# hucsmn/suffix_array

Measured on AMD Instinct MI355X. Metric: input MB/s indexed (SA build), higher is better.
Workload: dtype u8; 1 GPU; c3_english_256m: 268435456 bytes per GPU, seed base + rank, one independent text per GPU; n_bytes=268435456, sigma=57, symbols_per_key=13, refinement_rounds=9, text_rounds=0, radix_passes=25, unresolved_after_initial_sort=199000237

## Files before the change

### suffix_array_amd/csrc/host/pipeline.hpp

```cpp
#pragma once
#include "support.hpp"
#include "tuning.hpp"
#include "pool.hpp"

#include <functional>

namespace sa {

constexpr int SORT_MAX_WG = 1024;
constexpr int BK_TOP_BITS_MAX = 18;
constexpr uint32_t BK_BUCKETS_MAX = 1u << BK_TOP_BITS_MAX;
static_assert(32 - 16 <= BK_MAX_LBITS, "two 8-bit passes inside a bucket");
constexpr size_t GRAM_MAX_ENTRIES = (size_t)1 << 24;
static_assert(GROUP_CAP_MAX == GS_CAP, "Tuning clamps SA_AMD_GROUP_CAP to the kernel's cap");

#ifdef SA_AMD_DIAG
typedef void (*DownsweepFn)(const uint64_t *, const uint32_t *, uint64_t *, uint32_t *, uint32_t *,
                            const uint32_t *, int64_t, int, uint32_t, int64_t, int);
struct SortVariant { int threads, items, wg_per_cu; DownsweepFn fn; const char *name; };
static const SortVariant sort_variants[] = {
    { 1024, 8, 2, k_radix_downsweep_wcl<1024, 8, 16, 1, false, uint64_t, 4>, "carry-completed lines 1024x8 + LDS prefetch of half of the next tile's keys (default)" },
    { 1024, 8, 2, k_radix_downsweep_wcl<1024, 8>, "carry-completed lines 1024x8" },
    { 512, 16, 1, k_radix_downsweep_wcl<512, 16>, "carry-completed lines 512x16" },
    { 1024, 8, 2, k_radix_downsweep_wcl<1024, 8, 8>, "carry 1024x8, granule 8" },
// ... 24 lines not shown
}

#else
constexpr int N_SORT_VARIANTS = 1;
#endif

struct SortScratch {
    uint32_t *spine;
    uint32_t *digit_tot;
    unsigned long long *status;
    uint32_t *err;
};

struct Workspace {
    uint64_t *keysA, *keysB, *keysC;
    uint32_t *valsA, *valsB, *isa, *U0, *U1, *G0, *G1;
    uint32_t *spine, *digit_tot, *tcnt, *thead, *tnext, *hist, *total, *chg, *has_isa;
    uint8_t *packed;
    uint8_t *gram_flags;
    uint4 *gram_table;
    uint32_t *surv_bits, *surv_cnt, *todo_bits, *ft_cnt, *ft_head;
    unsigned long long *os_status;
    uint32_t *os_err;
    uint32_t *bk_start;
    uint32_t *early_bits, *early_cnt;
    SortScratch ss;
    size_t bytes, bytes2;
};

static Workspace carve(void *base, int64_t n, size_t cap = ~(size_t)0, void *base2 = nullptr)
{
    Workspace w;
    const size_t N = (size_t)(n > 0 ? n : 1);
    size_t off = 0, off2 = 0;
    auto take = [&](size_t b) {
        if (off + b <= cap) { size_t o = off; off = align_up(off + b, 256); return (char *)base + o; }
        size_t o = off2; off2 = align_up(off2 + b, 256); return (char *)base2 + o;
    };
    const size_t rr_tiles = (size_t)ceil_div((int64_t)N, RR_TILE);
    const size_t ft_tiles = (size_t)ceil_div((int64_t)N, FT_TILE) + 1;
    const size_t gram_entries = N < GRAM_MAX_ENTRIES ? N : GRAM_MAX_ENTRIES;
    w.spine = (uint32_t *)take((size_t)RADIX * SORT_MAX_WG * 4);
    w.digit_tot = (uint32_t *)take(RADIX * 4);
    w.os_status = (unsigned long long *)take(((size_t)ceil_div((int64_t)N, OS_MIN_TILE) + 1) * RADIX * 8);
    w.os_err = (uint32_t *)take(256);
    w.hist = (uint32_t *)take(256 * 4);
    w.total = (uint32_t *)take(256);
    w.chg = (uint32_t *)take((size_t)RR_CHG_COUNTERS * 32 * 4);
    w.tcnt = (uint32_t *)take(rr_tiles * 4);
    w.thead = (uint32_t *)take(rr_tiles * 4);
    w.tnext = (uint32_t *)take(rr_tiles * 4);
    w.surv_cnt = (uint32_t *)take(rr_tiles * 4);
    w.ft_cnt = (uint32_t *)take(ft_tiles * 4);
    w.ft_head = (uint32_t *)take(ft_tiles * 4);
    w.bk_start = (uint32_t *)take(((size_t)BK_BUCKETS_MAX + 1) * 4);
    w.early_cnt = (uint32_t *)take(((N + 1 + EARLY_TILE - 1) / EARLY_TILE + 8) * 4);
    w.gram_table = (uint4 *)take((gram_entries / 64 + 1) * 16);
    w.has_isa = (uint32_t *)take((N + 31) / 32 * 4);
    w.surv_bits = (uint32_t *)take((N + 31) / 32 * 4);
    w.todo_bits = (uint32_t *)take((N + 31) / 32 * 4);
    w.early_bits = (uint32_t *)take(((N + 1 + 31) / 32 + EARLY_THREADS) * 4);
    w.gram_flags = (uint8_t *)take(gram_entries + 64);
    w.packed = (uint8_t *)take(N / 2 + 64);
    w.keysA = (uint64_t *)take((N + 64) * 8);
    w.keysB = (uint64_t *)take((N + 64) * 8);
    w.valsA = (uint32_t *)take(N * 4);
    w.valsB = (uint32_t *)take(N * 4);
    w.isa = (uint32_t *)take(N * 4);
// ... 965 lines not shown
    int64_t threshold = 0;
    std::function<void(hipEvent_t)> start;
    std::function<int64_t()> stop;
    bool started = false;
    int64_t m_snap = 0;
    int64_t covered = 0;
    int64_t holes = 0;
    const uint32_t *d_bits = nullptr, *d_tile_off = nullptr, *d_holes = nullptr;
    hipEvent_t ev = nullptr;
};

struct DeviceBuild {
    const uint8_t *dT;
    uint32_t *dSA, *SA;
    int64_t n;
    hipStream_t st;
    Tuning tn;
    Workspace w;
    sa_amd_stats local;
    EarlyDownload *early = nullptr;
    bool trace = false;
    double trace_t = 0;
    double lap() { const double t = now_ms(), d = t - trace_t; trace_t = t; return d; }
    bool timing_only() const
    {
#ifdef SA_AMD_DIAG
        return tn.timing_only_initial_sort;
#else
        return false;
#endif
    }
    KeyParams P, Ptext;
    int sigma = 0, key_bits = 0, g_bits = 0, top_shift = 0;
    bool force_dense = false, text_ok = false, local_ok = false, probe_dense = false;
    SortResult sr;
    const uint32_t *sorted32 = nullptr;
    int bucket_top_bits = 0;
    bool flat_text = false;
    bool bucket_finished = false;
    uint64_t *sorted0 = nullptr;
    uint32_t *Ucur = nullptr, *Unext = nullptr, *Gcur = nullptr, *Gnext = nullptr, *Vcur = nullptr;
    uint64_t *rkA = nullptr, *rkB = nullptr;
    int64_t tiles = 0, m = 0, depth = 0;
    uint32_t m32 = 0;
    bool lists_ready = false, finished32 = false, fused64 = false, sparse = false;
    bool isa_tail_ranks = false;
// ... 482 lines not shown
        m = m32;
        local.unresolved_after_initial = m;
        if (timing_only()) m = 0;
        }
        return SA_AMD_OK;
    }

    int finish_top32_ties()
    {
        int rc = SA_AMD_OK; (void)rc;
        if (!finished32 && top_shift && m > 0) {
            rkA = (sr.keys == w.keysA) ? w.keysB : w.keysA;
            rkB = w.keysC;
            PROF(KC_RR_APPLY, n, st, hipLaunchKernelGGL((k_rr_apply<true, false, 1, uint32_t>), dim3((unsigned)tiles), dim3(RR_THREADS), 0, st,
                                                        sorted32, (const uint32_t *)SA, (const uint32_t *)nullptr, n,
                                                        (const uint32_t *)w.tcnt, (const uint32_t *)w.thead, SA, w.isa, Ucur, Gcur, Vcur, 0u,
                                                        w.has_isa, 0, (uint64_t *)nullptr, (uint32_t *)nullptr, (const uint32_t *)w.total, 0, (const uint32_t *)nullptr, 0, (uint32_t *)nullptr));
            uint32_t *Valt = (Vcur == w.valsA) ? w.valsB : w.valsA;
            Refined rf;
            KeySrc K = KeySrc(); K.mode = KS_LOWKEY; K.kb = top_shift;
            rc = refine_list(rkA, rkB, Vcur, Valt, Ucur, Gcur, Unext, Gnext, m, n, dT, P, K, g_bits, &local_ok, w, st, &local, &rf, tn);
            if (rc) return rc;
            tiles = ceil_div(m, RR_TILE);
            PROF(KC_RR_COUNT, m, st, hipLaunchKernelGGL((k_rr_count<false>), dim3((unsigned)tiles), dim3(RR_THREADS), 0, st, rf.keys,
                                                        (const uint32_t *)Ucur, m, w.tcnt, w.thead, 0, (uint32_t *)nullptr, 0));
            PROF(KC_RR_SCAN, tiles, st, hipLaunchKernelGGL((k_rr_scan), dim3(1), dim3(SPINE_THREADS), 0, st, w.tcnt, w.thead, tiles, w.total));
            PROF(KC_RR_APPLY, m, st, hipLaunchKernelGGL((k_rr_apply<false, true, 3>), dim3((unsigned)tiles), dim3(RR_THREADS), 0, st,
                                                        rf.keys, rf.vals, (const uint32_t *)Ucur, m, (const uint32_t *)w.tcnt,
                                                        (const uint32_t *)w.thead, SA, w.isa, Unext, Gnext, rf.vnext, (uint32_t)n,
                                                        (uint32_t *)nullptr, 0, (uint64_t *)nullptr, (uint32_t *)nullptr,
                                                        (const uint32_t *)w.total, 0, (const uint32_t *)nullptr, 0, (uint32_t *)nullptr));
            { const int rcw = read_words(&m32, w.total, 4, st); if (rcw) return rcw; }
            m = m32;
            uint32_t *t;
            t = Ucur; Ucur = Unext; Unext = t;
            t = Gcur; Gcur = Gnext; Gnext = t;
            Vcur = rf.vnext;
            lists_ready = true;
            local.unresolved_after_initial = m;
        }
        return SA_AMD_OK;
    }

    int rank_setup_and_text_rounds()
    {
        int rc = SA_AMD_OK; (void)rc;
        key2_bits = bit_length((uint64_t)(2 * n));
        const int64_t sparse_div = tn.sparse_div;
        const int64_t sparse_limit = n / sparse_div;
        sparse = false;
        const bool dense_first = m > 0 && !lists_ready && (force_dense || (!text_ok && m > sparse_limit) || (probe_dense && m > sparse_limit));
        if (m > 0 && dense_first) {
            isa_tail_ranks = !tn.no_first_tail;
            if (isa_tail_ranks)
// ... 39 lines not shown
                PROF(KC_RR_APPLY, n, st, hipLaunchKernelGGL((k_rr_apply<true, false, 1>), dim3((unsigned)tiles), dim3(RR_THREADS), 0, st,
                                                            (const uint64_t *)sorted0, (const uint32_t *)SA, (const uint32_t *)nullptr, n,
                                                            (const uint32_t *)w.tcnt, (const uint32_t *)w.thead, SA, w.isa, Ucur, Gcur, Vcur, 0u,
                                                            w.has_isa, 0, (uint64_t *)nullptr, (uint32_t *)nullptr, (const uint32_t *)w.total, 0, (const uint32_t *)nullptr, 0, (uint32_t *)nullptr));
            }
            bool progressing = true;

            bool counters_clear = false;
            while (text_ok && s_sym > 0 && m > sparse_limit && local.text_rounds < tn.max_text_rounds && progressing) {
                if ((rc = early_maybe_start())) return rc;
                const int64_t m_before = m;
                uint32_t *Valt = (Vcur == w.valsA) ? w.valsB : w.valsA;
                Refined rf;
                KeySrc K = KeySrc(); K.mode = KS_TEXT; K.h = depth; K.s = s_sym; K.kb = tkb;
                RoundCtl ctl;
                ctl.defer = prev_clean && local_ok && !tn.no_defer;
                ctl.counters_clear = counters_clear;
                rc = refine_list(rkA, rkB, Vcur, Valt, Ucur, Gcur, Unext, Gnext, m, n, dT, Ptext, K, g_bits, &local_ok, w, st, &local, &rf, tn, false, nullptr, &ctl);
                if (rc) return rc;
                uint32_t words[RC_WORDS];
                for (int attempt = 0; ; ++attempt) {
                    const uint32_t *gate = ctl.deferred ? (const uint32_t *)(w.total + RC_FLAGGED) : (const uint32_t *)nullptr;
                    tiles = ceil_div(m, RR_TILE);
                    PROF(KC_RR_COUNT, m, st, hipLaunchKernelGGL((k_rr_count<false>), dim3((unsigned)tiles), dim3(RR_THREADS), 0, st, rf.keys,
                                                                (const uint32_t *)Ucur, m, w.tcnt, w.thead, 0, (uint32_t *)nullptr, 0, gate));
                    PROF(KC_RR_SCAN, tiles, st, hipLaunchKernelGGL((k_rr_scan_round), dim3(2), dim3(SPINE_THREADS), 0, st, w.tcnt, w.thead, tiles, w.total,
                                                                   (uint32_t *)nullptr, (uint32_t *)nullptr, w.total + RC_BIG_LISTED, gate));
                    PROF(KC_RR_APPLY, m, st, hipLaunchKernelGGL((k_rr_apply<false, true, 3>), dim3((unsigned)tiles), dim3(RR_THREADS), 0, st,
                                                                rf.keys, rf.vals, (const uint32_t *)Ucur, m, (const uint32_t *)w.tcnt,
                                                                (const uint32_t *)w.thead, SA, w.isa, Unext, Gnext, rf.vnext,
                                                                (uint32_t)n, (uint32_t *)nullptr, 0, (uint64_t *)nullptr, (uint32_t *)nullptr,
                                                                (const uint32_t *)w.total, 0, (const uint32_t *)nullptr, 0, (uint32_t *)nullptr, gate));
                    { const int rcw = read_words(words, w.total, sizeof(words), st); if (rcw) return rcw; }
                    if (!ctl.deferred) break;
                    if (words[RC_FLAGGED] == 0) { ctl.m_flagged = 0; local.locally_sorted += m; break; }
                    if (attempt > 0) return SA_AMD_EINTERNAL;
                    uint32_t tot[RC_WORDS];
                    memcpy(tot, words, sizeof(tot));
                    ctl.resume_tot = tot; ctl.defer = false; ctl.deferred = false;
                    rc = refine_list(rkA, rkB, Vcur, Valt, Ucur, Gcur, Unext, Gnext, m, n, dT, Ptext, K, g_bits, &local_ok, w, st, &local, &rf, tn, false, nullptr, &ctl);
                    if (rc) return rc;
                    ctl.resume_tot = nullptr;
                }
                prev_clean = ctl.m_flagged == 0;
                counters_clear = true;
                uint32_t *Vnext = rf.vnext;
                m32 = words[0];
                m = m32;
                uint32_t *t;
                t = Ucur; Ucur = Unext; Unext = t;
                t = Gcur; Gcur = Gnext; Gnext = t;
                Vcur = Vnext;
                depth += s_sym;
                local.text_rounds++;
                local.rounds++;
// ... 47 lines not shown
            KeySrc K = KeySrc();
            K.mode = sparse ? KS_SPARSE : KS_RANK; K.h = h; K.kb = key2_bits; K.isa = w.isa;
            if (!local_ok && !tn.no_local_sort && m * 2 < m_local_off) local_ok = true;
            const bool retry_local = !local_ok && ++rounds_local_off >= 3;
            K.iters = (!sparse && local_ok && chase_ok) ? (m >= tn.chase_big_min ? tn.chase_big : tn.chase) : 1;
            if (K.iters > 1) K.mode = KS_CHASE;
            K.has_isa = w.has_isa; K.sorted_keys = sorted0; K.sorted_top32 = sorted32; K.sa = SA; K.depth = depth_text; K.top_shift = top_shift;
            Refined rf;
            if (local_ok) { m_local_off = m; rounds_local_off = 0; }
            const int64_t expect = (!parent_tail || m < changed_prev) ? m : changed_prev;
            const bool bin = !sparse && binned(n, expect, tn);
            RoundCtl ctl;
            ctl.defer = prev_clean && !bin && local_ok && !tn.no_defer;
            ctl.skip_big = all_small;
            ctl.counters_clear = counters_clear;
            rc = refine_list(rkA, rkB, Vcur, Valt, Ucur, Gcur, Unext, Gnext, m, n, dT, P, K, g_bits, &local_ok, w, st, &local, &rf, tn, retry_local, &split_rest, &ctl);
            if (rc) return rc;
            uint32_t words[64 + RR_CHG_COUNTERS * 32];
            for (int attempt = 0; ; ++attempt) {
                if (retry_local && rf.m_global < m) { m_local_off = m; rounds_local_off = 0; }
                const uint64_t *keysS = rf.keys; const uint32_t *valsS = rf.vals; uint32_t *Vnext = rf.vnext;
                const uint32_t *gate = ctl.deferred ? (const uint32_t *)(w.total + RC_FLAGGED) : (const uint32_t *)nullptr;
                tiles = ceil_div(m, RR_TILE);
                if (sparse)
                    PROF(KC_RR_COUNT, m, st, hipLaunchKernelGGL((k_rr_count<false>), dim3((unsigned)tiles), dim3(RR_THREADS), 0, st, keysS, Ucur, m, w.tcnt,
                                       w.thead, 0, (uint32_t *)nullptr, 0, gate));
                else
                    PROF(KC_RR_COUNT, m, st, hipLaunchKernelGGL((k_rr_count<false, uint64_t, true>), dim3((unsigned)tiles), dim3(RR_THREADS), 0, st, keysS, Ucur, m,
                                       w.tcnt, w.thead, 0, w.tnext, key2_bits, gate));
                PROF(KC_RR_SCAN, tiles, st, hipLaunchKernelGGL((k_rr_scan_round), dim3(2), dim3(SPINE_THREADS), 0, st, w.tcnt, w.thead, tiles, w.total,
                                                               sparse ? (uint32_t *)nullptr : w.tnext, sparse ? (uint32_t *)nullptr : w.chg, w.total + RC_BIG_LISTED, gate));
                if (sparse) {
                    PROF(KC_RR_APPLY, m, st, hipLaunchKernelGGL((k_rr_apply<false, true, 1>), dim3((unsigned)tiles), dim3(RR_THREADS), 0, st,
                                                                keysS, valsS, Ucur, m, w.tcnt, w.thead, SA, w.isa, Unext, Gnext, Vnext,
                                                                (uint32_t)n, w.has_isa, key2_bits, (uint64_t *)nullptr, (uint32_t *)nullptr, (const uint32_t *)w.total, 0, (const uint32_t *)nullptr, 0, (uint32_t *)nullptr, gate));
                } else if (bin) {
                    uint64_t *pk = (keysS == rkA) ? rkB : rkA;
                    PROF(KC_RR_APPLY, m, st, hipLaunchKernelGGL((k_rr_apply<false, true, 2>), dim3((unsigned)tiles), dim3(RR_THREADS), 0, st,
                                                                keysS, valsS, Ucur, m, w.tcnt, w.thead, SA, w.isa, Unext, Gnext, Vnext,
                                                                (uint32_t)n, (uint32_t *)nullptr, key2_bits, pk, Gcur, (const uint32_t *)w.total, 0,
                                                                (const uint32_t *)w.tnext, parent_tail ? 1 : 0, w.chg, (const uint32_t *)nullptr, sa_final));
                    { const int rcw = read_words(words, w.total, sizeof(words), st); if (rcw) return rcw; }
                    int64_t pairs = 0;
                    for (int c = 0; c < RR_CHG_COUNTERS; ++c) pairs += words[64 + c * 32];
                    if (pairs > 0) {
                        rc = scatter_binned((uint32_t *)pk, Gcur, (uint32_t *)keysS, (uint32_t *)valsS, pairs, n, w, st, &local, tn);
                        if (rc) return rc;
                    }
                    break;
                } else {
                    PROF(KC_RR_APPLY, m, st, hipLaunchKernelGGL((k_rr_apply<false, true, 0>), dim3((unsigned)tiles), dim3(RR_THREADS), 0, st,
                                                                keysS, valsS, Ucur, m, w.tcnt, w.thead, SA, w.isa, Unext, Gnext, Vnext,
                                                                (uint32_t)n, (uint32_t *)nullptr, key2_bits, (uint64_t *)nullptr,
                                                                (uint32_t *)nullptr, (const uint32_t *)w.total, 0,
                                                                (const uint32_t *)w.tnext, parent_tail ? 1 : 0, w.chg, gate, sa_final));
                }
                { const int rcw = read_words(words, w.total, sparse ? (size_t)RC_WORDS * 4 : sizeof(words), st); if (rcw) return rcw; }
                if (!ctl.deferred) break;
                if (words[RC_FLAGGED] == 0) {
                    ctl.m_flagged = 0;
                    ctl.big_listed = ctl.skip_big ? -1 : (int64_t)words[RC_BIG_LISTED_SAVED];
                    rf.m_global = words[RC_BIG_ORDERED_SAVED];
                    local.locally_sorted += m;
                    break;
                }
                if (attempt > 0) return SA_AMD_EINTERNAL;
                uint32_t tot[RC_WORDS];
                memcpy(tot, words, sizeof(tot));
                ctl.resume_tot = tot; ctl.defer = false; ctl.deferred = false;
                rc = refine_list(rkA, rkB, Vcur, Valt, Ucur, Gcur, Unext, Gnext, m, n, dT, P, K, g_bits, &local_ok, w, st, &local, &rf, tn, retry_local, &split_rest, &ctl);
                if (rc) return rc;
                ctl.resume_tot = nullptr;
                ++deferred_misses;
            }
            uint32_t *Vnext = rf.vnext;
            prev_clean = ctl.m_flagged == 0;
            if (prev_clean && (ctl.big_listed == 0 || m <= GS_CAP)) all_small = true;
            counters_clear = true;
            {
// ... 39 lines not shown
        PROF(KC_MISC, 1, st, hipLaunchKernelGGL((k_set_u32), dim3(1), dim3(1), 0, st, dSA, 0u));
        HIP_TRY(hipStreamSynchronize(st));
        if (stats) *stats = local;
        return SA_AMD_OK;
    }
    B.w = dWork2 ? carve(dWork, n, (size_t)work_bytes, dWork2) : carve(dWork, n);
    const Workspace &w = B.w;
    if ((int64_t)w.bytes > work_bytes || (int64_t)w.bytes2 > work2_bytes) return SA_AMD_EINVAL;
    if (n <= tn.small_max) {
        if (n <= SM_LITE_SINGLE_N)
            PROF(KC_MISC, n, st, hipLaunchKernelGGL((k_small_sa_lite), dim3(1), dim3(SM_LITE_THREADS), 0, st, dT, dSA, (int)n, w.total));
        else
            PROF(KC_MISC, n, st, hipLaunchKernelGGL((k_small_sa), dim3(1), dim3(SM_THREADS), 0, st, dT, dSA, (int)n, w.total));
        uint32_t rounds = 0;
        { const int rcw = read_words(&rounds, w.total, 4, st); if (rcw) return rcw; }
        local.rounds = (int)rounds;
        local.readbacks = g_readbacks;
        g_prof.resolve();
        g_last_stats = local;
        if (stats) *stats = local;
        return SA_AMD_OK;
    }
    HIP_TRY(hipMemsetAsync(w.os_err, 0, 16, st));
    int rc;
    if ((rc = B.geometry_and_probes())) return rc;
    if (!B.unary_done) {
    if ((rc = B.initial_sort())) return rc;
    if ((rc = B.first_round_from_sorted_keys())) return rc;
    if ((rc = B.group_heads())) return rc;
    if ((rc = B.finish_top32_ties())) return rc;
    if ((rc = B.rank_setup_and_text_rounds())) return rc;
    if ((rc = B.doubling_rounds())) return rc;
    }
    if ((rc = B.early_finish())) return rc;
    hipLaunchKernelGGL(k_set_u32, dim3(1), dim3(1), 0, st, dSA, (uint32_t)n);
    LAUNCH_CHECK(st);
    {
        uint32_t gave_up[4] = { 0, 0, 0, 0 };
        const int rcw = read_words(gave_up, w.os_err, 16, st); if (rcw) return rcw;
        if (gave_up[0] || gave_up[3]) return SA_AMD_EINTERNAL;
    }
    local.readbacks = g_readbacks;
    if (B.trace) fprintf(stderr, "suffix_array_amd: %d blocking read-backs in this build (%d rounds deferred their mid-round count and had to run the global sort after all)\n", g_readbacks, B.deferred_misses);
    g_prof.resolve();
    g_last_stats = local;
    if (stats) *stats = local;
// ... 5 lines not shown
```

### suffix_array_amd/csrc/host/tuning.hpp

```cpp
#pragma once
#include <cstdlib>
#include <cstdint>
#include <atomic>

namespace sa {

constexpr int64_t SPARSE_DIV_DEFAULT = 64;
constexpr int GROUP_CAP_MAX = 1024;

constexpr int UNBWT_SPACING_DEFAULT = 256;
constexpr int UNBWT_SPACING_MAX = 65536;
constexpr int UNBWT_SPACING_MIN = 4;
constexpr int UNBWT_CAP_DEFAULT = 4096;
constexpr int UNBWT_CAP_MAX = 1 << 24;
constexpr int UNBWT_RESTART_WALKS = 64;

inline bool env_flag(const char *name)
{
    const char *e = getenv(name);
    return e && *e && !(e[0] == '0' && e[1] == 0);
}

inline int64_t env_int(const char *name, int64_t def, int64_t lo, int64_t hi)
{
// ... 14 lines not shown
struct Tuning {
    int sort_variant = 0;
    int sort32_variant = 0;
    int key_bits_max = 64;
    int group_cap = GROUP_CAP_MAX;
    int64_t sparse_div = SPARSE_DIV_DEFAULT;
    bool sparse_div_set = false;
    bool force_dense = false;
    bool no_text_rounds = false;
    bool no_local_sort = false;
    bool no_top32 = false;
    bool force_top32 = false;
    bool no_fused_finish = false;
    bool fused64 = false;
    bool no_packed_text = false;
    bool no_binned_isa = false;
    bool binned_isa_always = false;
    bool no_run_skip = false;
    int64_t run_skip_min = (int64_t)1 << 25;
    int64_t dense_rekey_min = (int64_t)1 << 22;
    bool no_first_tail = false;
    bool sa_every_round = false;
    bool setup_key_copy = false;
    bool no_repeat_probe = false;
    int64_t binned_min = (int64_t)1 << 26;
    int chase = 7;
    int chase_big = 3;
    int64_t chase_big_min = (int64_t)1 << 23;
    int scatter_levels = 0;
    int max_text_rounds = 4;
    bool no_split = false;
    int64_t split_min = (int64_t)1 << 22;
    int64_t split_group_min = (int64_t)1 << 15;
    bool no_gram_keys = false;
    int64_t gram_min_n = (int64_t)1 << 22;
    int gram_g = 0;
    int gram_tail_max = 8;
    int top32_partners_x100 = 50;
    int top32_collisions_x100 = 400;
    int64_t top32_probe_min_n = (int64_t)1 << 21;
    int small_max = 8192;
    bool no_onesweep = false;
    int onesweep_flags = 0;
    int onesweep64_shape = 0;
    int onesweep32_shape = 0;
    bool no_unary_shortcut = false;
// ... 80 lines not shown
        t.count_next_below_n = env_int("SA_AMD_COUNT_NEXT_BELOW_N", 393216, 0, (int64_t)1 << 40);
        t.no_unary_shortcut = env_flag("SA_AMD_NO_UNARY_SHORTCUT");

        t.no_text_keys = env_flag("SA_AMD_NO_TEXT_KEYS");
        t.no_value_bits = env_flag("SA_AMD_NO_VALUE_BITS");
        t.no_bucket_sort = env_flag("SA_AMD_NO_BUCKET_SORT");
        t.bucket_min_n = env_int("SA_AMD_BUCKET_MIN_N", (int64_t)1 << 25, 1, (int64_t)1 << 40);
        t.no_bucket_finish = env_flag("SA_AMD_NO_BUCKET_FINISH");
        t.bucket_finish_always = env_flag("SA_AMD_BUCKET_FINISH_ALWAYS");
        t.bucket_bits = (int)env_int("SA_AMD_BUCKET_BITS", 0, 0, 18);
        if (t.bucket_bits != 16 && t.bucket_bits != 18) t.bucket_bits = 0;
        t.bucket_shape = (int)env_int("SA_AMD_BUCKET_SHAPE", -1, -1, 64);
#ifdef SA_AMD_DIAG
        t.sample_sort = env_flag("SA_AMD_SAMPLE_SORT");
        t.sample_merge = env_flag("SA_AMD_SAMPLE_MERGE");
        t.sample_sort_min_n = env_int("SA_AMD_SAMPLE_SORT_MIN_N", (int64_t)1 << 26, (int64_t)1 << 17, (int64_t)1 << 40);
        t.sample_log = (int)env_int("SA_AMD_SAMPLE_LOG", 0, 0, 24);
        if (t.sample_log != 0 && t.sample_log < 16) t.sample_log = 16;
        t.timing_only_initial_sort = env_flag("SA_AMD_TIMING_ONLY_INITIAL_SORT");
        {
            const int r = g_rerank_routes.load(std::memory_order_relaxed);
            t.sa_every_round = (r & 1) != 0;
            t.setup_key_copy = (r & 2) != 0;
        }
#endif
        return t;
    }
};

constexpr size_t STAGE_BYTES = (size_t)16 << 20;

struct HostTuning {
    int small_max;
    int copy_threads;
    size_t staged_min;
    bool prefault;
    int prefault_keep;
    bool prefault_wait;
    int64_t early_div;
    size_t early_min;
    size_t early_chunk;
    int64_t early_wait;
    bool reduced;
    bool lanes;
    int64_t lanes_min_n;
    bool kernel_d2h;
// ... 28 lines not shown
```

### suffix_array_amd/csrc/kernels/onesweep.hpp

```cpp
#pragma once
#include "common.hpp"
#include "radix_sort.hpp"

namespace sa {

constexpr int OS_NSEG = 8;
constexpr int OS_LB = 3;
struct __attribute__((packed, aligned(4))) Words4 { uint32_t x, y, z, w; };
constexpr int OS_MIN_TILE = 4096;

__device__ __forceinline__ unsigned os_xcc_id()
{
    return (unsigned)__builtin_amdgcn_s_getreg((3 << 11) | 20) & 7u;
}

typedef __attribute__((address_space(1))) unsigned long long os_gu64;

__device__ __forceinline__ uint32_t text_key32(const uint8_t *__restrict__ T, int64_t n, int64_t i)
{
    if (i + 8 <= n) {
        const uintptr_t a = (uintptr_t)(T + i);
        const uint32_t *W = (const uint32_t *)(a & ~(uintptr_t)3);
        const uint32_t lo = W[0], hi = W[1];
        const uint32_t le = __builtin_amdgcn_alignbyte(hi, lo, (uint32_t)(a & 3u));
        return __builtin_bswap32(le);
    }
    uint32_t k = 0;
#pragma unroll
    for (int b = 0; b < 4; ++b) k = (k << 8) | (i + b < n ? (uint32_t)T[i + b] : 0u);
    return k;
}

__global__ __launch_bounds__(SORT_THREADS) void k_text_upsweep32(const uint8_t *__restrict__ T, int64_t n, uint32_t *__restrict__ counts,
                                                                 int shift, uint32_t dmask, int64_t chunk_elems, int G, int split, int64_t sub_elems)
{
    __shared__ uint32_t h[SORT_WAVES][512];
    for (int i = threadIdx.x; i < SORT_WAVES * 512; i += SORT_THREADS) (&h[0][0])[i] = 0;
    __syncthreads();
    uint32_t *mine = h[wave_id()];
// ... 456 lines not shown
```

### suffix_array_amd/csrc/kernels/rerank.hpp

```cpp
#pragma once
#include "common.hpp"

namespace sa {

constexpr int RR_THREADS = 1024;
constexpr int RR_ITEMS = 8;
constexpr int RR_TILE = RR_THREADS * RR_ITEMS;

constexpr int RR_WAVE_ELEMS = WAVE * RR_ITEMS;

struct WaveGroups { uint64_t head[RR_ITEMS], tied[RR_ITEMS], valid[RR_ITEMS], phead[RR_ITEMS]; };

__device__ __forceinline__ uint64_t shfl64(uint64_t v, int src)
{
    return ((uint64_t)(uint32_t)__shfl((int)(uint32_t)(v >> 32), src, WAVE) << 32) | (uint32_t)__shfl((int)(uint32_t)v, src, WAVE);
}

template <typename KeyT, bool PARENTS = false>
__device__ __forceinline__ WaveGroups rr_wave_classify(const KeyT *__restrict__ keys, int64_t m, int64_t wbase, int key_shift, int g_shift = 0,
                                                       uint64_t *kout = nullptr)
{
    const int l = lane_id();
    uint64_t k[RR_ITEMS];
    WaveGroups g;
// ... 180 lines not shown
{
    rr_scan_body(tile_cnt, tile_head, tiles, out_total);
}

__global__ __launch_bounds__(SPINE_THREADS) void k_rr_scan_pair(uint32_t *__restrict__ cntA, uint32_t *__restrict__ headA, uint32_t *__restrict__ outA,
                                                                 uint32_t *__restrict__ cntB, uint32_t *__restrict__ headB, uint32_t *__restrict__ outB,
                                                                 int64_t tiles)
{
    if (blockIdx.x == 0) rr_scan_body(cntA, headA, tiles, outA);
    else rr_scan_body(cntB, headB, tiles, outB);
}

__global__ __launch_bounds__(SPINE_THREADS) void k_rr_scan_round(uint32_t *__restrict__ tile_cnt, uint32_t *__restrict__ tile_head, int64_t tiles,
                                                                  uint32_t *__restrict__ out_total, uint32_t *__restrict__ tile_first,
                                                                  uint32_t *__restrict__ changed_cnt, uint32_t *__restrict__ clear2,
                                                                  const uint32_t *__restrict__ gate)
{
    if (gate && *gate) return;
    if (blockIdx.x == 0) { rr_scan_body(tile_cnt, tile_head, tiles, out_total); return; }
    if (tile_first) rr_scan_next_body(tile_first, tiles, changed_cnt);
    if (threadIdx.x == 0 && clear2) { clear2[2] = clear2[0]; clear2[3] = clear2[1]; clear2[0] = 0u; clear2[1] = 0u; }
}

template <bool FIRST, bool WRITE_SA, int ISA_MODE, typename KeyT = uint64_t, bool FTAIL = false>
__global__ __launch_bounds__(RR_THREADS) void k_rr_apply(
    const KeyT *__restrict__ keys, const uint32_t *__restrict__ V, const uint32_t *__restrict__ U, int64_t m,
    const uint32_t *__restrict__ tile_cnt, const uint32_t *__restrict__ tile_head, uint32_t *__restrict__ SA,
    uint32_t *__restrict__ ISA, uint32_t *__restrict__ Uo, uint32_t *__restrict__ Go, uint32_t *__restrict__ Vo,
    uint32_t n_text, uint32_t *__restrict__ has_isa, int g_shift, uint64_t *__restrict__ pair_k,
    uint32_t *__restrict__ pair_v, const uint32_t *__restrict__ tile_total, int key_shift,
    const uint32_t *__restrict__ tile_next, int parent_tail, uint32_t *__restrict__ changed_cnt,
    const uint32_t *__restrict__ gate = nullptr,
    int sa_final = 0)
{
    constexpr bool SPARSE = ISA_MODE == 1;
    if (gate && *gate) return;
    constexpr bool TAIL = (FIRST ? FTAIL : true) && (ISA_MODE == 0 || ISA_MODE == 2);
    constexpr bool COUNT_CHANGED = TAIL && !FIRST;
    constexpr int NW = RR_THREADS / WAVE;
    __shared__ uint32_t wcnt[NW], whead[NW], wfirst[NW];
    __shared__ uint32_t s_chg;
    if (COUNT_CHANGED && threadIdx.x == 0) s_chg = 0;
    if (FIRST && !WRITE_SA && SPARSE) {
        const uint32_t here = tile_cnt[blockIdx.x];
        const uint32_t next = (blockIdx.x + 1 < gridDim.x) ? tile_cnt[blockIdx.x + 1] : *tile_total;
        if (next == here) return;
    }
    const int l = lane_id(), w = wave_id();
    const int64_t wbase = (int64_t)blockIdx.x * RR_TILE + (int64_t)w * RR_WAVE_ELEMS;
    const WaveGroups g = rr_wave_classify<KeyT, TAIL>(keys, m, wbase, key_shift, g_shift);
    uint32_t slot[RR_ITEMS], v[RR_ITEMS];
#pragma unroll
    for (int r = 0; r < RR_ITEMS; ++r) {
        const int64_t i = wbase + 64 * r + l;
        const bool in = i < m;
        slot[r] = FIRST ? (uint32_t)i : (in ? U[i] : 0u);
        v[r] = in ? V[i] : 0u;
    }
    {
        uint32_t cnt = 0, lasthead = 0;
#pragma unroll
        for (int r = 0; r < RR_ITEMS; ++r) {
            cnt += (uint32_t)__popcll(g.tied[r]);
            if (g.head[r]) lasthead = (uint32_t)__shfl((int)slot[r], 63 - __builtin_clzll(g.head[r]), WAVE) + 1u;
        }
        if (l == 0) { wcnt[w] = cnt; whead[w] = lasthead; wfirst[w] = TAIL ? rr_first_head_code(g, wbase, 0) : RR_NO_HEAD; }
    }
    __syncthreads();
    uint32_t run_cnt = tile_cnt[blockIdx.x], run_head = tile_head[blockIdx.x];
    for (int ww = 0; ww < w; ++ww) { run_cnt += wcnt[ww]; run_head = run_head > whead[ww] ? run_head : whead[ww]; }
    uint32_t next_code[RR_ITEMS];
    uint32_t n_changed = 0;
    if (TAIL) {
        uint32_t behind = tile_next[blockIdx.x];
        for (int ww = NW - 1; ww > w; --ww) behind = wfirst[ww] != RR_NO_HEAD ? wfirst[ww] : behind;
        if (behind == RR_NO_HEAD) behind = ((uint32_t)m << 1) | 1u;
#pragma unroll
        for (int r = RR_ITEMS - 1; r >= 0; --r) {
            next_code[r] = behind;
            if (g.head[r]) {
                const int b = __builtin_ctzll(g.head[r]);
                behind = ((uint32_t)(wbase + 64 * r + b) << 1) | (uint32_t)((g.phead[r] >> b) & 1ull);
            }
        }
    }
    const uint64_t le_mask = (l == 63) ? ~0ull : ((2ull << l) - 1ull);
    const uint64_t lt_mask = le_mask >> 1;
    auto code_behind = [&](int r) -> uint32_t {
        const uint64_t hgt = (l == 63) ? 0ull : (g.head[r] & (~0ull << (l + 1)));
        if (!hgt) return next_code[r];
        const int b = __builtin_ctzll(hgt);
        return ((uint32_t)(wbase + 64 * r + b) << 1) | (uint32_t)((g.phead[r] >> b) & 1ull);
    };
    constexpr bool PAIRS = COUNT_CHANGED && ISA_MODE == 2;
    uint64_t cmask[PAIRS ? RR_ITEMS : 1];
    uint32_t pair_off = 0;
    if (PAIRS) {
// ... 47 lines not shown
            } else if (ISA_MODE != 3 && ISA_MODE != 4 && v[r] < n_text) {
                if (changed) {
                    ISA[v[r]] = rank;
                    if (SPARSE) atomicOr(&has_isa[v[r] >> 5], 1u << (v[r] & 31u));
                }
            }
            if ((g.tied[r] >> l) & 1ull) {
                if (ISA_MODE == 4) {
                    ISA[slot[r]] = run - 1u;
                    atomicOr(&has_isa[slot[r] >> 5], 1u << (slot[r] & 31u));
                    atomicAdd(&pair_v[slot[r] / RR_TILE], 1u);
                } else {
                    Uo[off] = slot[r]; Go[off] = run - 1u; Vo[off] = v[r];
                }
            }
        }
        run_cnt += (uint32_t)__popcll(g.tied[r]);
        if (g.head[r]) run_head = (uint32_t)__shfl((int)slot[r], 63 - __builtin_clzll(g.head[r]), WAVE) + 1u;
        if (PAIRS) pair_off += (uint32_t)__popcll(cmask[r]);
    }
    if (COUNT_CHANGED && !PAIRS) {
        if (l == 0 && n_changed) atomicAdd(&s_chg, n_changed);
        __syncthreads();
        if (threadIdx.x == 0 && s_chg) atomicAdd(&changed_cnt[(blockIdx.x % RR_CHG_COUNTERS) * 32], s_chg);
    }
}

}
```

### suffix_array_amd/csrc/sa_diag.inc

```

SA_EXPORT int32_t sa_amd_debug_phase_cycles(uint64_t *out, int32_t count)
{
    unsigned long long h[16] = { 0 };
    if (hipMemcpyFromSymbol(h, HIP_SYMBOL(sa::g_phase_cycles), sizeof(h)) != hipSuccess) return SA_AMD_EHIP;
    for (int i = 0; i < count && i < 16; ++i) out[i] = h[i];
    unsigned long long z[16] = { 0 };
    (void)hipMemcpyToSymbol(HIP_SYMBOL(sa::g_phase_cycles), z, sizeof(z));
    return 16;
}

SA_EXPORT int32_t sa_amd_debug_group_sort_stamps(int32_t on)
{
    const int v = on ? 1 : 0;
    return hipMemcpyToSymbol(HIP_SYMBOL(sa::g_gs_stamp_on), &v, sizeof(v)) == hipSuccess ? SA_AMD_OK : SA_AMD_EHIP;
}

SA_EXPORT int32_t sa_amd_debug_rerank_routes(int32_t flags)
{
    return sa::g_rerank_routes.exchange(flags & 3);
}

SA_EXPORT int32_t sa_amd_debug_sort_variant_count(void) { return sa::N_SORT_VARIANTS; }
SA_EXPORT const char *sa_amd_debug_sort_variant_name(int32_t i)
{
    return (i >= 0 && i < sa::N_SORT_VARIANTS) ? sa::sort_variants[i].name : "";
}

SA_EXPORT int32_t sa_amd_test_sort_pairs(uint64_t *keys, uint32_t *vals, int64_t count, int32_t begin_bit, int32_t end_bit)
{
    using namespace sa;
    if (count < 0 || (count > 0 && (!keys || !vals)) || begin_bit < 0 || end_bit > 64) return SA_AMD_EINVAL;
    if (sa_amd_device_count() <= 0) return SA_AMD_ENODEVICE;
    if (count == 0) return SA_AMD_OK;
    const Tuning tn = Tuning::from_env(N_SORT_VARIANTS, N_SORT32_VARIANTS, N_OS_SHAPES64, N_OS_SHAPES32);
    const size_t N = (size_t)count;
    DevBuf dk, dv, dsp;
    int32_t rc;
    if ((rc = dk.alloc(N * 8 * 2))) return rc;
    if ((rc = dv.alloc(N * 4 * 2))) return rc;
    if ((rc = dsp.alloc(((size_t)RADIX * SORT_MAX_WG + RADIX) * 4))) return rc;
    uint64_t *k = dk.as<uint64_t>(); uint32_t *v = dv.as<uint32_t>(), *spine = dsp.as<uint32_t>();
    HIP_TRY(hipMemcpy(k, keys, N * 8, hipMemcpyHostToDevice));
// ... 227 lines not shown
```

Baseline: 5609 MB/s.

## Fuse rerank count/scan/apply into a single-pass kernel with decoupled lookback

Replaces the three-kernel rerank sequence (per-tile count, spine scan, apply) in the non-first list rounds with one kernel. That kernel takes dynamic tile tickets and computes each tile's prefix through a decoupled lookback over epoch-tagged status words. Run-start and run-end carries across tile boundaries come from wave-parallel searches over the sorted keys. This removes two launches per round and a pass over the keys, at the cost of serialized lookback spinning, extra boundary searches and a last-block cleanup of the control words.

```diff
diff --git a/suffix_array_amd/csrc/host/pipeline.hpp b/suffix_array_amd/csrc/host/pipeline.hpp
--- a/suffix_array_amd/csrc/host/pipeline.hpp
+++ b/suffix_array_amd/csrc/host/pipeline.hpp
@@ -70,6 +70,9 @@
     uint32_t *surv_bits, *surv_cnt, *todo_bits, *ft_cnt, *ft_head;
     unsigned long long *os_status;
     uint32_t *os_err;
+    uint32_t *rr_ctl;
+    unsigned long long *rr_status;
+    size_t rr_lb_bytes;
     uint32_t *bk_start;
     uint32_t *early_bits, *early_cnt;
     SortScratch ss;
@@ -92,6 +95,9 @@
     w.digit_tot = (uint32_t *)take(RADIX * 4);
     w.os_status = (unsigned long long *)take(((size_t)ceil_div((int64_t)N, OS_MIN_TILE) + 1) * RADIX * 8);
     w.os_err = (uint32_t *)take(256);
+    w.rr_lb_bytes = (size_t)RR1_CTL_WORDS * 4 + (rr_tiles + 1) * 8;
+    w.rr_ctl = (uint32_t *)take(w.rr_lb_bytes);
+    w.rr_status = (unsigned long long *)(w.rr_ctl + RR1_CTL_WORDS);
     w.hist = (uint32_t *)take(256 * 4);
     w.total = (uint32_t *)take(256);
     w.chg = (uint32_t *)take((size_t)RR_CHG_COUNTERS * 32 * 4);
@@ -1103,6 +1109,13 @@
     bool trace = false;
     double trace_t = 0;
     double lap() { const double t = now_ms(), d = t - trace_t; trace_t = t; return d; }
+    uint32_t rr_epoch = 0;
+    RrOnePass one_pass(uint32_t *clear2)
+    {
+        RrOnePass p;
+        p.status = w.rr_status; p.ctl = w.rr_ctl; p.err = w.os_err; p.out_total = w.total; p.clear2 = clear2; p.epoch = ++rr_epoch;
+        return p;
+    }
     bool timing_only() const
     {
 #ifdef SA_AMD_DIAG
@@ -1631,6 +1644,12 @@
             rc = refine_list(rkA, rkB, Vcur, Valt, Ucur, Gcur, Unext, Gnext, m, n, dT, P, K, g_bits, &local_ok, w, st, &local, &rf, tn);
             if (rc) return rc;
             tiles = ceil_div(m, RR_TILE);
+            if (!tn.rerank_three_kernels)
+                PROF(KC_RR_APPLY, m, st, hipLaunchKernelGGL((k_rr_apply1<3>), dim3((unsigned)tiles), dim3(RR_THREADS), 0, st,
+                                                            rf.keys, rf.vals, (const uint32_t *)Ucur, m, SA, w.isa, Unext, Gnext, rf.vnext, (uint32_t)n,
+                                                            (uint32_t *)nullptr, 0, 0, (uint32_t *)nullptr, (const uint32_t *)nullptr, 0,
+                                                            one_pass((uint32_t *)nullptr)));
+            else {
             PROF(KC_RR_COUNT, m, st, hipLaunchKernelGGL((k_rr_count<false>), dim3((unsigned)tiles), dim3(RR_THREADS), 0, st, rf.keys,
                                                         (const uint32_t *)Ucur, m, w.tcnt, w.thead, 0, (uint32_t *)nullptr, 0));
             PROF(KC_RR_SCAN, tiles, st, hipLaunchKernelGGL((k_rr_scan), dim3(1), dim3(SPINE_THREADS), 0, st, w.tcnt, w.thead, tiles, w.total));
@@ -1639,6 +1658,7 @@
                                                         (const uint32_t *)w.thead, SA, w.isa, Unext, Gnext, rf.vnext, (uint32_t)n,
                                                         (uint32_t *)nullptr, 0, (uint64_t *)nullptr, (uint32_t *)nullptr,
                                                         (const uint32_t *)w.total, 0, (const uint32_t *)nullptr, 0, (uint32_t *)nullptr));
+            }
             { const int rcw = read_words(&m32, w.total, 4, st); if (rcw) return rcw; }
             m = m32;
             uint32_t *t;
@@ -1724,6 +1744,11 @@
                 for (int attempt = 0; ; ++attempt) {
                     const uint32_t *gate = ctl.deferred ? (const uint32_t *)(w.total + RC_FLAGGED) : (const uint32_t *)nullptr;
                     tiles = ceil_div(m, RR_TILE);
+                    if (!tn.rerank_three_kernels)
+                        PROF(KC_RR_APPLY, m, st, hipLaunchKernelGGL((k_rr_apply1<3>), dim3((unsigned)tiles), dim3(RR_THREADS), 0, st,
+                                                                    rf.keys, rf.vals, (const uint32_t *)Ucur, m, SA, w.isa, Unext, Gnext, rf.vnext, (uint32_t)n,
+                                                                    (uint32_t *)nullptr, 0, 0, (uint32_t *)nullptr, gate, 0, one_pass(w.total + RC_BIG_LISTED)));
+                    else {
                     PROF(KC_RR_COUNT, m, st, hipLaunchKernelGGL((k_rr_count<false>), dim3((unsigned)tiles), dim3(RR_THREADS), 0, st, rf.keys,
                                                                 (const uint32_t *)Ucur, m, w.tcnt, w.thead, 0, (uint32_t *)nullptr, 0, gate));
                     PROF(KC_RR_SCAN, tiles, st, hipLaunchKernelGGL((k_rr_scan_round), dim3(2), dim3(SPINE_THREADS), 0, st, w.tcnt, w.thead, tiles, w.total,
@@ -1733,6 +1758,7 @@
                                                                 (const uint32_t *)w.thead, SA, w.isa, Unext, Gnext, rf.vnext,
                                                                 (uint32_t)n, (uint32_t *)nullptr, 0, (uint64_t *)nullptr, (uint32_t *)nullptr,
                                                                 (const uint32_t *)w.total, 0, (const uint32_t *)nullptr, 0, (uint32_t *)nullptr, gate));
+                    }
                     { const int rcw = read_words(words, w.total, sizeof(words), st); if (rcw) return rcw; }
                     if (!ctl.deferred) break;
                     if (words[RC_FLAGGED] == 0) { ctl.m_flagged = 0; local.locally_sorted += m; break; }
@@ -1826,6 +1852,17 @@
                 const uint64_t *keysS = rf.keys; const uint32_t *valsS = rf.vals; uint32_t *Vnext = rf.vnext;
                 const uint32_t *gate = ctl.deferred ? (const uint32_t *)(w.total + RC_FLAGGED) : (const uint32_t *)nullptr;
                 tiles = ceil_div(m, RR_TILE);
+                const bool one = !tn.rerank_three_kernels && !bin;
+                if (one) {
+                    if (sparse)
+                        PROF(KC_RR_APPLY, m, st, hipLaunchKernelGGL((k_rr_apply1<1>), dim3((unsigned)tiles), dim3(RR_THREADS), 0, st,
+                                                                    keysS, valsS, Ucur, m, SA, w.isa, Unext, Gnext, Vnext, (uint32_t)n, w.has_isa, key2_bits, 0,
+                                                                    (uint32_t *)nullptr, gate, 0, one_pass(w.total + RC_BIG_LISTED)));
+                    else
+                        PROF(KC_RR_APPLY, m, st, hipLaunchKernelGGL((k_rr_apply1<0>), dim3((unsigned)tiles), dim3(RR_THREADS), 0, st,
+                                                                    keysS, valsS, Ucur, m, SA, w.isa, Unext, Gnext, Vnext, (uint32_t)n, (uint32_t *)nullptr, key2_bits,
+                                                                    parent_tail ? 1 : 0, w.chg, gate, sa_final, one_pass(w.total + RC_BIG_LISTED)));
+                } else {
                 if (sparse)
                     PROF(KC_RR_COUNT, m, st, hipLaunchKernelGGL((k_rr_count<false>), dim3((unsigned)tiles), dim3(RR_THREADS), 0, st, keysS, Ucur, m, w.tcnt,
                                        w.thead, 0, (uint32_t *)nullptr, 0, gate));
@@ -1859,6 +1896,7 @@
                                                                 (uint32_t *)nullptr, (const uint32_t *)w.total, 0,
                                                                 (const uint32_t *)w.tnext, parent_tail ? 1 : 0, w.chg, gate, sa_final));
                 }
+                }
                 { const int rcw = read_words(words, w.total, sparse ? (size_t)RC_WORDS * 4 : sizeof(words), st); if (rcw) return rcw; }
                 if (!ctl.deferred) break;
                 if (words[RC_FLAGGED] == 0) {
@@ -1944,6 +1982,7 @@
         return SA_AMD_OK;
     }
     HIP_TRY(hipMemsetAsync(w.os_err, 0, 16, st));
+    HIP_TRY(hipMemsetAsync(w.rr_ctl, 0, w.rr_lb_bytes, st));
     int rc;
     if ((rc = B.geometry_and_probes())) return rc;
     if (!B.unary_done) {
diff --git a/suffix_array_amd/csrc/host/tuning.hpp b/suffix_array_amd/csrc/host/tuning.hpp
--- a/suffix_array_amd/csrc/host/tuning.hpp
+++ b/suffix_array_amd/csrc/host/tuning.hpp
@@ -60,6 +60,7 @@
     bool no_first_tail = false;
     bool sa_every_round = false;
     bool setup_key_copy = false;
+    bool rerank_three_kernels = false;
     bool no_repeat_probe = false;
     int64_t binned_min = (int64_t)1 << 26;
     int chase = 7;
@@ -186,6 +187,7 @@
             const int r = g_rerank_routes.load(std::memory_order_relaxed);
             t.sa_every_round = (r & 1) != 0;
             t.setup_key_copy = (r & 2) != 0;
+            t.rerank_three_kernels = (r & 4) != 0;
         }
 #endif
         return t;
diff --git a/suffix_array_amd/csrc/kernels/onesweep.hpp b/suffix_array_amd/csrc/kernels/onesweep.hpp
--- a/suffix_array_amd/csrc/kernels/onesweep.hpp
+++ b/suffix_array_amd/csrc/kernels/onesweep.hpp
@@ -15,6 +15,42 @@
 }
 
 typedef __attribute__((address_space(1))) unsigned long long os_gu64;
+
+__device__ __forceinline__ unsigned long long os_tag(uint32_t epoch, uint32_t flag) { return ((unsigned long long)(epoch * 4u + flag)) << 32; }
+
+__device__ __forceinline__ uint32_t os_lookback_excl(os_gu64 *status, int64_t t, uint32_t epoch, uint32_t own, uint32_t *err)
+{
+    const int l = (int)(threadIdx.x & (WAVE - 1));
+    const unsigned long long tagA = os_tag(epoch, 1u), tagI = os_tag(epoch, 2u);
+    uint32_t acc = 0;
+    if (t > 0) {
+        if (l == 0) __hip_atomic_store(status + t, tagA | (unsigned long long)own, __ATOMIC_RELAXED, __HIP_MEMORY_SCOPE_AGENT);
+        int64_t k = t - 1;
+        unsigned spins = 0;
+        while (k >= 0) {
+            const int64_t idx = k - l;
+            const unsigned long long x = idx >= 0 ? __hip_atomic_load(status + idx, __ATOMIC_RELAXED, __HIP_MEMORY_SCOPE_AGENT) : 0ull;
+            const unsigned long long tg = x & 0xffffffff00000000ull;
+            const bool isI = idx >= 0 && tg == tagI, isA = idx >= 0 && tg == tagA;
+            const unsigned long long bI = __ballot(isI), bR = __ballot(isI || isA);
+            const int firstI = bI ? __builtin_ctzll(bI) : 64, firstBad = ~bR ? __builtin_ctzll(~bR) : 64;
+            const bool done = firstI < firstBad;
+            const int take = done ? firstI + 1 : firstBad;
+            uint32_t v = l < take ? (uint32_t)x : 0u;
+#pragma unroll
+            for (int o = 1; o < WAVE; o <<= 1) v += (uint32_t)__shfl_xor((int)v, o, WAVE);
+            acc += v;
+            if (done) break;
+            k -= take;
+            if (take == 0) {
+                if (++spins > (1u << 22)) { if (l == 0) atomicAdd(err, 1u); break; }
+                __builtin_amdgcn_s_sleep(2);
+            }
+        }
+    }
+    if (l == 0) __hip_atomic_store(status + t, tagI | (unsigned long long)(acc + own), __ATOMIC_RELAXED, __HIP_MEMORY_SCOPE_AGENT);
+    return acc;
+}
 
 __device__ __forceinline__ uint32_t text_key32(const uint8_t *__restrict__ T, int64_t n, int64_t i)
 {
diff --git a/suffix_array_amd/csrc/kernels/rerank.hpp b/suffix_array_amd/csrc/kernels/rerank.hpp
--- a/suffix_array_amd/csrc/kernels/rerank.hpp
+++ b/suffix_array_amd/csrc/kernels/rerank.hpp
@@ -1,5 +1,6 @@
 #pragma once
 #include "common.hpp"
+#include "onesweep.hpp"
 
 namespace sa {
 
@@ -226,19 +227,75 @@
     if (threadIdx.x == 0 && clear2) { clear2[2] = clear2[0]; clear2[3] = clear2[1]; clear2[0] = 0u; clear2[1] = 0u; }
 }
 
-template <bool FIRST, bool WRITE_SA, int ISA_MODE, typename KeyT = uint64_t, bool FTAIL = false>
-__global__ __launch_bounds__(RR_THREADS) void k_rr_apply(
+constexpr int RR1_TICKET = 0, RR1_DONE = 1, RR1_CHG = 32;
+constexpr int RR1_CTL_WORDS = RR1_CHG + RR_CHG_COUNTERS * 32;
+struct RrOnePass {
+    unsigned long long *status = nullptr;
+    uint32_t *ctl = nullptr;
+    uint32_t *err = nullptr;
+    uint32_t *out_total = nullptr;
+    uint32_t *clear2 = nullptr;
+    uint32_t epoch = 0;
+};
+
+template <typename KeyT>
+__device__ __forceinline__ int64_t rr_run_start(const KeyT *__restrict__ keys, int64_t p, int key_shift)
+{
+    const int l = lane_id();
+    const uint64_t kp = (uint64_t)keys[p] >> key_shift;
+    int64_t lo = -1, hi = p, step = 1;
+    while (hi - lo > 1) {
+        const int64_t q = hi - (int64_t)(l + 1) * step;
+        const bool valid = q > lo;
+        const bool eq = valid && ((uint64_t)keys[q] >> key_shift) == kp;
+        const int c = __popcll(__ballot(eq)), nv = __popcll(__ballot(valid));
+        const int64_t h0 = hi;
+        hi = h0 - (int64_t)c * step;
+        if (c < nv) lo = h0 - (int64_t)(c + 1) * step;
+        step = (hi - lo - 1 + 63) / 64;
+    }
+    return hi;
+}
+
+template <typename KeyT>
+__device__ __forceinline__ int64_t rr_run_end(const KeyT *__restrict__ keys, int64_t m, int64_t p, int key_shift)
+{
+    const int l = lane_id();
+    const uint64_t kp = (uint64_t)keys[p] >> key_shift;
+    int64_t lo = p, hi = m, step = 1;
+    while (hi - lo > 1) {
+        const int64_t q = lo + (int64_t)(l + 1) * step;
+        const bool valid = q < hi;
+        const bool eq = valid && ((uint64_t)keys[q] >> key_shift) == kp;
+        const int c = __popcll(__ballot(eq)), nv = __popcll(__ballot(valid));
+        const int64_t l0 = lo;
+        lo = l0 + (int64_t)c * step;
+        if (c < nv) hi = l0 + (int64_t)(c + 1) * step;
+        step = (hi - lo - 1 + 63) / 64;
+    }
+    return hi;
+}
+
+template <bool FIRST, bool WRITE_SA, int ISA_MODE, typename KeyT, bool FTAIL, bool ONEPASS>
+__device__ __forceinline__ void rr_apply_tile(
     const KeyT *__restrict__ keys, const uint32_t *__restrict__ V, const uint32_t *__restrict__ U, int64_t m,
     const uint32_t *__restrict__ tile_cnt, const uint32_t *__restrict__ tile_head, uint32_t *__restrict__ SA,
     uint32_t *__restrict__ ISA, uint32_t *__restrict__ Uo, uint32_t *__restrict__ Go, uint32_t *__restrict__ Vo,
     uint32_t n_text, uint32_t *__restrict__ has_isa, int g_shift, uint64_t *__restrict__ pair_k,
     uint32_t *__restrict__ pair_v, const uint32_t *__restrict__ tile_total, int key_shift,
     const uint32_t *__restrict__ tile_next, int parent_tail, uint32_t *__restrict__ changed_cnt,
-    const uint32_t *__restrict__ gate = nullptr,
-    int sa_final = 0)
+    const uint32_t *__restrict__ gate, int sa_final, const RrOnePass &P)
 {
     constexpr bool SPARSE = ISA_MODE == 1;
+    static_assert(!ONEPASS || (!FIRST && ISA_MODE != 2 && ISA_MODE != 4), "the single-pass form covers the list rounds that do not pack pairs");
     if (gate && *gate) return;
+    __shared__ int64_t s_tile;
+    __shared__ uint32_t s_carry[3];
+    if (ONEPASS) {
+        if (threadIdx.x == 0) s_tile = (int64_t)atomicAdd(&P.ctl[RR1_TICKET], 1u);
+        __syncthreads();
+    }
+    const int64_t tile = ONEPASS ? s_tile : (int64_t)blockIdx.x;
     constexpr bool TAIL = (FIRST ? FTAIL : true) && (ISA_MODE == 0 || ISA_MODE == 2);
     constexpr bool COUNT_CHANGED = TAIL && !FIRST;
     constexpr int NW = RR_THREADS / WAVE;
@@ -246,12 +303,12 @@
     __shared__ uint32_t s_chg;
     if (COUNT_CHANGED && threadIdx.x == 0) s_chg = 0;
     if (FIRST && !WRITE_SA && SPARSE) {
-        const uint32_t here = tile_cnt[blockIdx.x];
-        const uint32_t next = (blockIdx.x + 1 < gridDim.x) ? tile_cnt[blockIdx.x + 1] : *tile_total;
+        const uint32_t here = tile_cnt[tile];
+        const uint32_t next = (tile + 1 < (int64_t)gridDim.x) ? tile_cnt[tile + 1] : *tile_total;
         if (next == here) return;
     }
     const int l = lane_id(), w = wave_id();
-    const int64_t wbase = (int64_t)blockIdx.x * RR_TILE + (int64_t)w * RR_WAVE_ELEMS;
+    const int64_t wbase = tile * RR_TILE + (int64_t)w * RR_WAVE_ELEMS;
     const WaveGroups g = rr_wave_classify<KeyT, TAIL>(keys, m, wbase, key_shift, g_shift);
     uint32_t slot[RR_ITEMS], v[RR_ITEMS];
 #pragma unroll
@@ -270,13 +327,44 @@
         }
         if (l == 0) { wcnt[w] = cnt; whead[w] = lasthead; wfirst[w] = TAIL ? rr_first_head_code(g, wbase, 0) : RR_NO_HEAD; }
     }
+    if (ONEPASS) {
+        const int64_t t0 = tile * RR_TILE;
+        const int64_t last = (t0 + RR_TILE < m ? t0 + RR_TILE : m) - 1;
+        if (w == 0) {
+            uint32_t carry = 0;
+            if (t0 > 0 && ((uint64_t)keys[t0 - 1] >> key_shift) == ((uint64_t)keys[t0] >> key_shift)) {
+                const int64_t s = rr_run_start<KeyT>(keys, t0 - 1, key_shift);
+                carry = U[s] + 1u;
+            }
+            if (l == 0) s_carry[1] = carry;
+        }
+        if (TAIL && w == NW - 1) {
+            const int64_t e = rr_run_end<KeyT>(keys, m, last, key_shift);
+            uint32_t code = RR_NO_HEAD;
+            if (e < m) code = ((uint32_t)e << 1) | (((((uint64_t)keys[e] >> key_shift) ^ ((uint64_t)keys[e - 1] >> key_shift)) >> g_shift) != 0ull ? 1u : 0u);
+            if (l == 0) s_carry[2] = code;
+        }
+    }
     __syncthreads();
-    uint32_t run_cnt = tile_cnt[blockIdx.x], run_head = tile_head[blockIdx.x];
+    if (ONEPASS) {
+        if (w == 0) {
+            uint32_t tot = l < NW ? wcnt[l] : 0u;
+#pragma unroll
+            for (int o = 1; o < NW; o <<= 1) tot += (uint32_t)__shfl_xor((int)tot, o, WAVE);
+            const uint32_t before = os_lookback_excl((os_gu64 *)P.status, tile, P.epoch, tot, P.err);
+            if (l == 0) {
+                s_carry[0] = before;
+                if ((tile + 1) * RR_TILE >= m) *P.out_total = before + tot;
+            }
+        }
+        __syncthreads();
+    }
+    uint32_t run_cnt = ONEPASS ? s_carry[0] : tile_cnt[tile], run_head = ONEPASS ? s_carry[1] : tile_head[tile];
     for (int ww = 0; ww < w; ++ww) { run_cnt += wcnt[ww]; run_head = run_head > whead[ww] ? run_head : whead[ww]; }
     uint32_t next_code[RR_ITEMS];
     uint32_t n_changed = 0;
     if (TAIL) {
-        uint32_t behind = tile_next[blockIdx.x];
+        uint32_t behind = ONEPASS ? s_carry[2] : tile_next[tile];
         for (int ww = NW - 1; ww > w; --ww) behind = wfirst[ww] != RR_NO_HEAD ? wfirst[ww] : behind;
         if (behind == RR_NO_HEAD) behind = ((uint32_t)m << 1) | 1u;
 #pragma unroll
@@ -370,8 +458,51 @@
     if (COUNT_CHANGED && !PAIRS) {
         if (l == 0 && n_changed) atomicAdd(&s_chg, n_changed);
         __syncthreads();
-        if (threadIdx.x == 0 && s_chg) atomicAdd(&changed_cnt[(blockIdx.x % RR_CHG_COUNTERS) * 32], s_chg);
-    }
-}
-
-}
+        if (threadIdx.x == 0 && s_chg) {
+            if (ONEPASS) {
+                const uint32_t was = atomicAdd(&P.ctl[RR1_CHG + (tile % RR_CHG_COUNTERS) * 32], s_chg);
+                asm volatile("s_waitcnt vmcnt(0)" : : "v"(was) : "memory");
+            } else
+                atomicAdd(&changed_cnt[(tile % RR_CHG_COUNTERS) * 32], s_chg);
+        }
+    }
+    if (ONEPASS && threadIdx.x == 0) {
+        const uint32_t tiles = (uint32_t)((m + RR_TILE - 1) / RR_TILE);
+        if (__hip_atomic_fetch_add(&P.ctl[RR1_DONE], 1u, __ATOMIC_RELAXED, __HIP_MEMORY_SCOPE_AGENT) == tiles - 1u) {
+            if (changed_cnt)
+                for (int c = 0; c < RR_CHG_COUNTERS; ++c)
+                    changed_cnt[c * 32] = __hip_atomic_exchange(&P.ctl[RR1_CHG + c * 32], 0u, __ATOMIC_RELAXED, __HIP_MEMORY_SCOPE_AGENT);
+            if (P.clear2) { P.clear2[2] = P.clear2[0]; P.clear2[3] = P.clear2[1]; P.clear2[0] = 0u; P.clear2[1] = 0u; }
+            __hip_atomic_store(&P.ctl[RR1_TICKET], 0u, __ATOMIC_RELAXED, __HIP_MEMORY_SCOPE_AGENT);
+            __hip_atomic_store(&P.ctl[RR1_DONE], 0u, __ATOMIC_RELAXED, __HIP_MEMORY_SCOPE_AGENT);
+        }
+    }
+}
+
+template <bool FIRST, bool WRITE_SA, int ISA_MODE, typename KeyT = uint64_t, bool FTAIL = false>
+__global__ __launch_bounds__(RR_THREADS) void k_rr_apply(
+    const KeyT *__restrict__ keys, const uint32_t *__restrict__ V, const uint32_t *__restrict__ U, int64_t m,
+    const uint32_t *__restrict__ tile_cnt, const uint32_t *__restrict__ tile_head, uint32_t *__restrict__ SA,
+    uint32_t *__restrict__ ISA, uint32_t *__restrict__ Uo, uint32_t *__restrict__ Go, uint32_t *__restrict__ Vo,
+    uint32_t n_text, uint32_t *__restrict__ has_isa, int g_shift, uint64_t *__restrict__ pair_k,
+    uint32_t *__restrict__ pair_v, const uint32_t *__restrict__ tile_total, int key_shift,
+    const uint32_t *__restrict__ tile_next, int parent_tail, uint32_t *__restrict__ changed_cnt,
+    const uint32_t *__restrict__ gate = nullptr,
+    int sa_final = 0)
+{
+    rr_apply_tile<FIRST, WRITE_SA, ISA_MODE, KeyT, FTAIL, false>(keys, V, U, m, tile_cnt, tile_head, SA, ISA, Uo, Go, Vo, n_text, has_isa, g_shift, pair_k,
+                                                                 pair_v, tile_total, key_shift, tile_next, parent_tail, changed_cnt, gate, sa_final, RrOnePass());
+}
+
+template <int ISA_MODE>
+__global__ __launch_bounds__(RR_THREADS) void k_rr_apply1(
+    const uint64_t *__restrict__ keys, const uint32_t *__restrict__ V, const uint32_t *__restrict__ U, int64_t m, uint32_t *__restrict__ SA,
+    uint32_t *__restrict__ ISA, uint32_t *__restrict__ Uo, uint32_t *__restrict__ Go, uint32_t *__restrict__ Vo, uint32_t n_text,
+    uint32_t *__restrict__ has_isa, int g_shift, int parent_tail, uint32_t *__restrict__ changed_cnt, const uint32_t *__restrict__ gate,
+    int sa_final, RrOnePass P)
+{
+    rr_apply_tile<false, true, ISA_MODE, uint64_t, false, true>(keys, V, U, m, nullptr, nullptr, SA, ISA, Uo, Go, Vo, n_text, has_isa, g_shift, nullptr,
+                                                                nullptr, nullptr, 0, nullptr, parent_tail, changed_cnt, gate, sa_final, P);
+}
+
+}
diff --git a/suffix_array_amd/csrc/sa_diag.inc b/suffix_array_amd/csrc/sa_diag.inc
--- a/suffix_array_amd/csrc/sa_diag.inc
+++ b/suffix_array_amd/csrc/sa_diag.inc
@@ -17,7 +17,7 @@
 
 SA_EXPORT int32_t sa_amd_debug_rerank_routes(int32_t flags)
 {
-    return sa::g_rerank_routes.exchange(flags & 3);
+    return sa::g_rerank_routes.exchange(flags & 7);
 }
 
 SA_EXPORT int32_t sa_amd_debug_sort_variant_count(void) { return sa::N_SORT_VARIANTS; }
```

New measurement: 5655 MB/s, median of 6. About the same (+0.8%).
